# skovaka/UNCALLED

Measured on NVIDIA H100. Metric: reads/sec mapped (E. coli, 4k-sample reads) at 1/2/4/8 H100 vs CPU ref, higher is better.
Workload: dtype f32/f64 events, u32 FM index

## Files before the change

uncalled_b200/csrc/unc_device.cuh:

```cuda
#pragma once
#include "unc_warp.cuh"

typedef uint8_t u8;
typedef uint16_t u16;
typedef uint32_t u32;
typedef int32_t i32;
typedef uint64_t u64;

#define UNC_NKMER 1024
#define UNC_KMASK 0x3FFu
#define UNC_SEED_LEN 22u
#define UNC_NGEN 24u
#define UNC_PATH_MASK 0x3FFFFFu
#define UNC_PATH_TAIL 0x200000u
#define UNC_INVALID 0x80000000u
#define UNC_BLK 32u


struct DevIndex {
    const uint4 *bwt;
    const u32 *sa;
    const u32 *sa_full;
    const uint2 *kmer_range;
    const float *lv_mean, *lv_var2, *lognorm;
// ... 671 lines not shown
        t.len_sum = f_add(t.len_sum, (float) ns.total_len);
        if (ns.total_len >= p.min_map_len && ns.total_len > t.max_map.total_len) t.max_map = ns;
        trk_insert_unique(t, ns, have_lb ? &lb : nullptr);
    }
    PT_TRK(t, 2)
}

UNC_DEV bool trk_get_final(const Tracker &t, const DevParams &p) {
    if (t.max_map.total_len < p.min_map_len || t.n_lens < 2) return false;
    float mean_len = f_div(t.len_sum, (float) t.n_live);
    float second_len = (float) t.top2;
    float sl = (float) t.max_map.total_len;
    return (p.min_mean_conf > 0 && f_div(sl, mean_len) >= p.min_mean_conf) ||
           (p.min_top_conf > 0 && f_div(sl, second_len) >= p.min_top_conf);
}

#define K2_CH_SLOTS 160u
#define K2_V2_DYN_BYTES (16u + K2_MAXSEG * (K2_CH_SLOTS * 8u + K2_CH_SLOTS))
#ifndef K2_MAXSEG
#define K2_MAXSEG 16u
#endif
#define K2_DYN_PER_CHUNK 8u
#define K2_SMEM_BYTES(maxp) (sizeof(K2Shared) + 16 + (size_t) (((maxp) + 31) / 32) * K2_DYN_PER_CHUNK + 32 + K2_V2_DYN_BYTES)
struct K2Tables {
    uint2 kmer_range[UNC_NKMER];
    float thresh[64];
};
struct K2V2 {
    K2V2Tab t;
    u32 kcnt[UNC_NKMER];
    u32 koff[UNC_NKMER];
    u32 kagg[UNC_NKMER];
    u32 fresh_cand[32], fresh_mask[32], fresh_before[32];
    u32 grab[2];
    u32 n_units;
    u16 mfirst[K2V2_MAX_MERGED];
#if defined(UNC_PHASE_TIMING) && !defined(UNC_EMUL)
    u32 pt_dur[4][K2_MAXSEG];
#endif
};
struct K2Shared {
    K2Tables tb;
    float probs[UNC_NKMER];
    u32 flags[32];
    u32 flags_prev[32];
    u32 sort_hist[256 * K2_MAXSEG];
    uint4 trk_dir[1024];
    u32 *bcnt, *ecnt;
    K2V2 v2;
    unsigned char *v2_stage;
    u32 bc[8];
    u32 n_rows[2];
    u32 verdict[2];
    u32 wk_overflow;
    u32 wl_cnt;
    u32 cnt_blocks, cnt_steps;
    u32 tot_children[2], tot_sources[2];
    DevWork work;
};

#include "unc_pdqsort.cuh"
#ifdef UNC_EMUL
static unsigned long g_emu_tie_stats[2];
#endif
UNC_DEV void write_source(uint4 *rec, uint2 *hist_e, u32 idx, u32 st, u32 en, u32 kmer, float prob) {
    rec[(size_t) idx * 2] = make_uint4(st, en, kmer | (1u << 16), 1u);
    rec[(size_t) idx * 2 + 1] = make_uint4(f2u(prob), f2u(prob), 0u, 0u);
    hist_e[idx] = make_uint2(f2u(prob), 0xFFFFFFFFu);
// ... 49 lines not shown
                } else right = mid;
            }
            rid = mid;
        }
        u64 rf_st = 0, rf_len = 0;
        if (rid >= 0) { rf_st = sa_st - B.seq_offsets[rid]; rf_len = B.seq_lens[rid]; }
        o.mapped = 1; o.fwd = fwd ? 1 : 0; o.rid = rid;
        o.rf_st = rf_st; o.rf_len = rf_len;
        o.rf_en = rf_st + ((u64) sc.ren_end - (u64) sc.ref_st + 5u);
        o.matches = (sc.total_len + 4u) & 0xFFFFu;
    }
    o.n_children = ((u64) sh->tot_children[1] << 32) | sh->tot_children[0];
    o.n_sources = ((u64) sh->tot_sources[1] << 32) | sh->tot_sources[0];
    o.n_seeds = n_seeds;
    o.n_occ_blocks = sh->cnt_blocks; o.n_sa_steps = sh->cnt_steps;
    B.out[r] = o;
}

#if defined(UNC_PHASE_TIMING) && !defined(UNC_EMUL)
UNC_DEV long long pt_clock() { long long v; asm volatile("mov.u64 %0, %%clock64;" : "=l"(v) :: "memory"); return v; }
#define PT_DECL unsigned long long pt_acc[32]; for (int _i = 0; _i < 32; _i++) pt_acc[_i] = 0; long long pt_t = pt_clock();
#define UNC_PT_TRACE_READ 40u
#define UNC_PT_TRACE_E0 60u
#define UNC_PT_TRACE_BYTES (8u * 16u * 32u * 8u)
#define PT_TRACE(ev, i, t) if ((B).dbg && r == UNC_PT_TRACE_READ && (ev) - UNC_PT_TRACE_E0 < 8u && (c_tid() & 31) == 0) \
        (B).dbg[(size_t) (B).n_reads * 64 + ((size_t) ((ev) - UNC_PT_TRACE_E0) * 16 + (c_tid() >> 5)) * 32 + (i)] = (unsigned long long) (t);
#define PT_MARK(i) { long long _n = pt_clock(); pt_acc[i] += (unsigned long long) (_n - pt_t); pt_t = _n; PT_TRACE(event_i, i, _n) }
#define PT_FLUSH(B, r) if ((B).dbg && (wt == 0 || wt == nwt - 32u)) { for (int _i = 0; _i < (wt == 0 ? 32 : 28); _i++) (B).dbg[(size_t) (r) * 64 + (wt == 0 ? 0 : 32) + _i] = pt_acc[_i]; }
#define PT_FENCE c_sync_sub(1, (int) nwt);
#define PT_WDECL long long pt_w0 = 0;
#define PT_WB pt_w0 = pt_clock();
#define PT_WE(ph) if (lane == 0) v2->pt_dur[ph][ww] = (u32) (pt_clock() - pt_w0);
#define PT_WARR(ph) if (lane == 0) v2->pt_dur[ph][ww] = (u32) pt_clock(); w_sync(); s_atomic_max(&v2->pt_dur[ph][ww], (u32) pt_clock());
#define PT_WREL(ph) if (lane == 0 && *(volatile u32 *) &v2->grab[0] != 0xFFFFFFFFu) { const long long _t = pt_clock(); v2->pt_dur[ph][ww] = (u32) _t; PT_TRACE(event_i, 30, _t) }
#define PT_WLAG(ph, s_last, s_first) if (wt == 0) { const u32 _now = (u32) pt_clock(); u32 _mn = 0xFFFFFFFFu, _mx = 0; for (u32 _w = 0; _w < nwk; _w++) { \
        const u32 _d = _now - *(volatile u32 *) &v2->pt_dur[ph][_w]; _mn = _d < _mn ? _d : _mn; _mx = _d > _mx ? _d : _mx; } pt_acc[s_last] += _mn; pt_acc[s_first] += _mx; }
#define PT_WTRK(ph, s) if (wt == 0) pt_acc[s] += (u32) pt_clock() - *(volatile u32 *) &v2->pt_dur[ph][K2_MAXSEG - 2 + (event_i & 1u)];
#define PT_WR(ph, s_max, s_mean) if (wt == 0) { u32 _mx = 0, _sm = 0; for (u32 _w = 0; _w < nwk; _w++) { const u32 _d = *(volatile u32 *) &v2->pt_dur[ph][_w]; \
        _mx = _d > _mx ? _d : _mx; _sm += _d; } pt_acc[s_max] += _mx; pt_acc[s_mean] += _sm / nwk; }
#else
#define PT_DECL
#define PT_MARK(i)
#define PT_FLUSH(B, r)
#define PT_FENCE
#define PT_WDECL
#define PT_WB
#define PT_WE(ph)
#define PT_WARR(ph)
#define PT_WLAG(ph, s_last, s_first)
#define PT_WTRK(ph, s)
#define PT_WREL(ph)
#define PT_WR(ph, s_max, s_mean)
#endif

template <bool STREAM>
UNC_DEV void unc_k2_tracker(const DevIndex &ix, const DevParams &p, const DevBatch &B, const DevWork &W,
                            K2Shared *sh, u32 r, u32 n_first, u32 n_limit) {
    const int lane = w_lane();
    Tracker trk;
    trk.blocks = W.clu; trk.dir_glob = W.dir; trk.max_blocks = W.max_blocks;
    trk.dir = sh->trk_dir; trk.dir_cap = (u32) (sizeof(sh->trk_dir) / sizeof(uint4));
    trk_reset(trk);
    DevMapState *ms = nullptr;
    if (STREAM) {
        ms = B.mstate + B.chan[r];
        if (ms->started) {
            trk.nb = ms->t_nb; trk.n_alloc = ms->t_n_alloc; trk.n_live = ms->t_n_live; trk.n_lens = ms->t_n_lens;
// ... 147 lines not shown
```

uncalled_b200/csrc/unc_k2v2.cuh:

```cuda
#pragma once

#define K2V2_STAGE_BYTES (K2_CH_SLOTS * 8u + K2_CH_SLOTS)


UNC_DEV void unc_occ2_build_block(const uint4 *bwt, u32 j, uint4 *out) {
    const uint4 *p = bwt + ((size_t) (j >> 1) << 2);
    const uint4 b0 = p[0], b1 = p[1];
    uint4 cnt = make_uint4(b0.x, b0.z, b1.x, b1.z);
    const uint4 lo = p[2], hi = p[3];
    if (j & 1u) {
        const u32 w[4] = {lo.x, lo.y, lo.z, lo.w};
        for (int i = 0; i < 4; i++) {
            const u32 h = w[i] >> 1, m = 0x55555555u;
            const u32 c3 = (u32) d_popc(h & w[i] & m), c2 = (u32) d_popc(h & ~w[i] & m), c1 = (u32) d_popc(~h & w[i] & m);
            cnt.x += 16u - c1 - c2 - c3; cnt.y += c1; cnt.z += c2; cnt.w += c3;
        }
    }
    out[(size_t) j * 2] = cnt;
    out[(size_t) j * 2 + 1] = (j & 1u) ? hi : lo;
}

UNC_DEV void unc_occ2_all(const uint4 cnt, const uint4 sym, u32 p, u32 o[4]) {
    u32 c1 = 0, c2 = 0, c3 = 0;
#pragma unroll
// ... 90 lines not shown
                }
                src[j] = key;
            }
        }
        w_sync();
    }
}

struct K2V2Walk {
    bool dup, begin_v, after_v, seed;
    u32 as, ae;
    u32 m_b, m_a, m_seed;
};
UNC_DEV K2V2Walk k2v2_walk(const uint4 cur, u32 nx, u32 ny, bool a, bool has_next, bool head, bool first, bool use_carry,
                           u32 carry_mx, bool prob_ok, uint2 kr, u32 *mx_last) {
    const int lane = w_lane();
    K2V2Walk r;
    r.dup = has_next && nx == cur.x && ny == cur.y;
    u32 mx = a ? cur.y : 0u;
    bool hd = head || !a;
    for (int d = 1; d < 32; d <<= 1) {
        const u32 omx = w_shfl_up(mx, d), ohd = w_shfl_up(hd ? 1u : 0u, d);
        if (lane >= d && !hd) { mx = omx > mx ? omx : mx; hd = ohd != 0; }
    }
    if (use_carry) mx = mx > carry_mx ? mx : carry_mx;
    *mx_last = w_shfl(mx, 31);
    r.begin_v = a && first && prob_ok && kr.x <= cur.x - 1u;
    r.as = mx + 1u;
    r.ae = has_next ? nx - 1u : kr.y;
    r.after_v = a && !r.dup && prob_ok && r.as <= r.ae;
    r.seed = a && !r.dup && (cur.w & 1u);
    r.m_b = w_ballot(r.begin_v); r.m_a = w_ballot(r.after_v); r.m_seed = w_ballot(r.seed);
    return r;
}

struct K2V2Pack {
    bool a;
    u32 bl;
    u32 start, pos, n;
};
UNC_DEV K2V2Pack k2v2_next_pack(u32 cnt, u32 P, u32 *remaining) {
    const int lane = w_lane();
    const int s = d_ffs(*remaining) - 1;
    const u32 Ps = w_shfl(P, s);
    const bool fits = ((*remaining >> lane) & 1u) && (P + cnt - Ps <= 32u);
    const u32 in_pack = w_ballot(fits);
    *remaining &= ~in_pack;
    const int e = 31 - d_clz(in_pack);
    const u32 T = w_shfl(P + cnt, e) - Ps;
    K2V2Pack k;
    k.a = (u32) lane < T;
    k.bl = (u32) s; k.start = 0;
    u32 m = in_pack;
    while (m) {
        const int b = d_ffs(m) - 1;
        m &= m - 1;
        const u32 sb = w_shfl(P, b) - Ps;
        if ((u32) lane >= sb) { k.bl = (u32) b; k.start = sb; }
    }
    k.pos = (u32) lane - k.start;
    k.n = w_shfl(cnt, (int) k.bl);
    return k;
}
UNC_DEV u32 k2v2_segmask(u32 start, u32 n) { return (n >= 32u ? 0xFFFFFFFFu : ((1u << n) - 1u)) << start; }

UNC_DEV u32 k2v2_slot(u32 rank) { return ((rank & 31u) << 5) | (rank >> 5); }
// ... 1 lines not shown
UNC_DEV uint2 *k2v2_stage(K2Shared *sh, u32 ww) {
    const u32 off = (u32) (sh->v2_stage - (unsigned char *) sh) + ww * K2V2_STAGE_BYTES;
    return (uint2 *) ((unsigned char *) sh + off);
}

UNC_DEV void k2v2_add64(u32 *w, u32 v) {
    const u64 s = (((u64) w[1] << 32) | w[0]) + v;
    w[0] = (u32) s; w[1] = (u32) (s >> 32);
}

UNC_DEV u32 k2v2_grab(u32 *counter) {
    u32 g = 0;
    if (w_lane() == 0) g = s_atomic_add(counter, 1u);
    return w_shfl(g, 0);
}

UNC_DEV void k2v2_sort_small(uint4 *keys, u32 n, uint4 *sst) {
    const int lane = w_lane();
    const bool a = (u32) lane < n;
    uint4 k = make_uint4(0, 0, 0, 0);
    if (a) k = keys[lane];
    u32 rnk = 0;
    const u32 kf = k2v2_fkey(k.z), kr_ = k.w >> 14;
    for (u32 j = 0; j < n; j++) {
        const u32 jx = w_shfl(k.x, (int) j), jy = w_shfl(k.y, (int) j), jf = w_shfl(kf, (int) j), jr = w_shfl(kr_, (int) j);
        if (k2v2_less_pre(jx, jy, jf, jr, k.x, k.y, kf, kr_)) rnk++;
    }
    if (a) sst[rnk] = k;
    w_sync();
    if (a) keys[lane] = sst[lane];
    w_sync();
}

struct K2V2Emit {
    uint4 *next; uint2 *hist_e; u32 *onext; uint2 *rlist;
    u32 S0, nc, maxp, n_ended_rows, rl_cap, pos0;
    u32 src_before, seeds_before;
};
template <bool EMIT>
UNC_DEV u32 k2v2_walk_merged(const DevIndex &ix, K2Shared *sh, const uint4 *keys, u32 n, u32 moff, float source_prob,
                             const K2V2Emit &E, u32 *pend_steps, u32 *pend_blocks, uint4 *sst) {
    K2V2 *v2 = &sh->v2;
    const u32 lane = (u32) w_lane();
    u32 nsrc = 0, nseed = 0, prev_sub = 0xFFFFFFFFu, un_st = 1, un_en = 0;
  for (u32 g0 = 0; g0 < n; g0 += 32u) {
    const u32 cnt = n - g0 < 32u ? n - g0 : 32u;
    if (lane < cnt) sst[lane] = keys[g0 + lane];
    if (lane == 0 && g0 + cnt < n) sst[32] = keys[g0 + cnt];
    w_sync();
    if (lane == 0)
    for (u32 j = 0; j < cnt; j++) {
        const u32 i = g0 + j;
        const uint4 cur = sst[j];
        const u32 sub = (cur.w >> 6) & 0xFFu, kmer = v2->t.mk[moff + sub];
        const uint2 kr = sh->tb.kmer_range[kmer];
        const float pk = sh->probs[kmer];
        const bool ok = pk >= source_prob;
        if (sub != prev_sub) {
            if (!EMIT && v2->mfirst[moff + sub] == 0xFFFFu) v2->mfirst[moff + sub] = (u16) nsrc;
            if (ok) {
                if (kr.x <= cur.x - 1u) {
                    const u32 sidx = E.src_before + nsrc;
                    if (EMIT && E.nc + sidx < E.maxp) {
                        write_source(E.next, E.hist_e, E.S0 + E.nc + sidx, kr.x, cur.x - 1u, kmer, pk);
                        E.onext[E.nc + sidx] = E.S0 + E.nc + sidx;
                    }
                    nsrc++;
                }
                un_st = cur.y + 1u; un_en = kr.y;
            }
        }
        prev_sub = sub;
        const bool has_next = i + 1u < n;
        uint4 nxt = make_uint4(0, 0, 0, 0);
        if (has_next) nxt = sst[j + 1u];
        const bool dup = has_next && nxt.x == cur.x && nxt.y == cur.y;
        const u32 rec = cur.w >> 14;
        if (EMIT) E.onext[E.pos0 + i] = rec | (dup ? UNC_INVALID : 0u);
        if (dup) continue;
        if (ok) {
            u32 src_st = un_st, src_en = un_en;
            if (has_next && ((nxt.w >> 6) & 0xFFu) == sub) {
                src_en = nxt.x - 1u;
                if (un_st <= nxt.y) un_st = nxt.y + 1u;
            }
            if (src_st <= src_en) {
                const u32 sidx = E.src_before + nsrc;
                if (EMIT && E.nc + sidx < E.maxp) {
                    write_source(E.next, E.hist_e, E.S0 + E.nc + sidx, src_st, src_en, kmer, pk);
                    E.onext[E.nc + sidx] = E.S0 + E.nc + sidx;
                }
                nsrc++;
            }
        }
        if (cur.w & 1u) {
            if (EMIT) {
                d_atomic_or(&((u32 *) (E.next + (size_t) rec * 2))[3], 0x80000000u);
                const u32 ri = E.n_ended_rows + E.seeds_before + nseed;
                if (ri < E.rl_cap) E.rlist[ri] = make_uint2(ix.seq_len - unc_sa_lookup(ix, cur.x, pend_steps, pend_blocks), (cur.w >> 1) & 0x1Fu);
                else sh->wk_overflow = 1;
            }
            nseed++;
        }
    }
    w_sync();
  }
    return w_shfl(nsrc | (nseed << 16), 0);
}

UNC_DEV void k2v2_bucket_offsets(K2V2 *v2) {
    const u32 lane = (u32) w_lane();
    u32 sum = 0;
#pragma unroll 1
    for (u32 j = 0; j < 32; j++) sum += v2->kcnt[j * 32u + lane];
    u32 tot, run = w_exscan(sum, &tot);
#pragma unroll 1
    for (u32 j = 0; j < 32; j++) {
        const u32 sl = j * 32u + lane, v = v2->kcnt[sl];
        v2->koff[sl] = run;
        v2->kcnt[sl] = run;
        run += v;
    }
}

UNC_DEV bool k2v2_exact_order(K2Shared *sh, const DevWork &W, u32 nc, u32 maxp, u32 wt, u32 nwt) {
    uint4 *ckA = W.ckey, *ckB = W.ckey + maxp;
    for (u32 i = wt; i + 1u < nc; i += nwt) {
        const uint4 k0 = ckA[i], k1 = ckA[i + 1u];
        if (!pq_less(k0, k1) && !pq_less(k1, k0)) *(volatile u32 *) &sh->bc[5] = 1u;
    }
    c_sync_sub(1, (int) nwt);
#ifdef UNC_EMUL
    if (wt == 0) { g_emu_tie_stats[0]++; g_emu_tie_stats[1] += sh->bc[5]; }
#endif
    if (!*(volatile u32 *) &sh->bc[5]) return false;
    for (u32 i = wt; i < nc; i += nwt) {
        const uint4 k = ckA[i];
        const u32 ci = k.w >> 14;
        ckB[sh->bcnt[ci / K2_CH_SLOTS] + ci % K2_CH_SLOTS] = k;
    }
    c_sync_sub(1, (int) nwt);
    if (wt == 0 && !unc_pdq_sort(ckB, nc, W.cks, ((maxp + 31u) >> 5) * K2_CH_SLOTS)) s_atomic_or(&sh->wk_overflow, 1u);
    c_sync_sub(1, (int) nwt);
    for (u32 i = wt; i < nc; i += nwt) ckA[i] = ckB[i];
    K2V2 *v2 = &sh->v2;
    if (wt == 0) { v2->grab[0] = 0; v2->n_units = 0; }
    for (u32 m = wt; m < K2V2_MAX_MERGED; m += nwt) v2->mfirst[m] = 0xFFFFu;
    c_sync_sub(1, (int) nwt);
    return true;
}

template <bool STREAM, bool EXACT, bool FLAGS>
UNC_DEV void unc_k2_workers_v2(const DevIndex &ix, const DevParams &p, const DevBatch &B, const DevWork &W,
                               K2Shared *sh, u32 r, u32 n_first, u32 n_limit) {
    const int lane = w_lane();
    const u32 wt = (u32) c_tid() - 32u, nwt = (u32) c_nthreads() - 32u;
    const u32 ww = wt >> 5, nwk = nwt >> 5;
    const K2Tables *tb = &sh->tb;
    K2V2 *v2 = &sh->v2;
    const u32 maxp = p.max_paths;
    const u32 S0 = ((maxp + 31u) >> 5) * K2_CH_SLOTS;
    const size_t gen_recs = (size_t) S0 + maxp;
    const float source_prob = tb->thresh[0];
    u32 my_blocks = 0, my_steps = 0, pend_blocks = 0, pend_steps = 0;
    u32 prev_size = 0, gen = 0, event_i = n_first;
    if (STREAM) {
        const DevMapState *ms = B.mstate + B.chan[r];
        if (ms->started) { prev_size = ms->prev_size; gen = ms->gen; }
    }
    if (wt == 0) { sh->tot_children[0] = sh->tot_children[1] = 0; sh->tot_sources[0] = sh->tot_sources[1] = 0; }
    const u32 lt = w_lanemask_lt();
    PT_DECL
    PT_WDECL

    for (; event_i < n_limit; event_i++) {
        PT_MARK(9)
        const float event = f_add(f_mul(B.scale[r], B.events[(size_t) r * B.ev_stride + (event_i - n_first)]), B.shift[r]);
        PT_MARK(7)

        if (FLAGS && wt < 32u) sh->flags_prev[wt] = sh->flags[wt];
        for (u32 k = wt; k < UNC_NKMER; k += nwt) {
            sh->probs[k] = unc_match_prob(event, d_ldg(ix.lv_mean + k), d_ldg(ix.lv_var2 + k), d_ldg(ix.lognorm + k));
            v2->kcnt[k] = 0; v2->kagg[k] = 0;
        }
        for (u32 j = ww; j < 32; j += nwk) {
            const u32 k = j * 32 + (u32) lane;
            const float pk = unc_match_prob(event, d_ldg(ix.lv_mean + k), d_ldg(ix.lv_var2 + k), d_ldg(ix.lognorm + k));
            const uint2 kr = tb->kmer_range[k];
            const u32 m = w_ballot(pk >= source_prob && kr.x <= kr.y);
            if (lane == 0) v2->fresh_cand[j] = m;
        }
        if (wt == 0) { v2->grab[0] = 0; v2->grab[1] = 0; v2->n_units = 0; }
        if (EXACT && wt == 0) sh->bc[5] = 0;
        if (wt < K2V2_MAX_MERGED) v2->mfirst[wt] = 0xFFFFu;
        PT_MARK(0)
        c_sync_sub(1, (int) nwt);
        PT_FENCE
        PT_MARK(16)


        const u32 nch_prev = (prev_size + 31u) >> 5;
        {
            const uint4 *prev = W.paths + (size_t) gen * gen_recs * 2;
            uint4 *next = W.paths + (size_t) (gen ^ 1u) * gen_recs * 2, *cks = W.cks;
            uint2 *hist_e = W.hist + (size_t) (event_i % UNC_NGEN) * gen_recs;
            const u32 *oprev = W.order + (size_t) gen * maxp;
            uint2 *stage_r = k2v2_stage(sh, ww);
            u8 *stage_m = (u8 *) (stage_r + K2_CH_SLOTS);
            u32 oi_n = UNC_INVALID, oi_nn = UNC_INVALID; uint4 q0_n = make_uint4(0, 0, 0, 0); uint2 q1_n = make_uint2(0, 0);
            if (ww < nch_prev) {
                const u32 pi = ww * 32u + (u32) lane;
                if (pi < prev_size) oi_n = oprev[pi];
                if (!(oi_n & UNC_INVALID)) { const uint4 *pr = prev + (size_t) oi_n * 2; q0_n = pr[0]; q1_n = *(const uint2 *) (pr + 1); }
            }
            if (ww + nwk < nch_prev) {
                const u32 pi = (ww + nwk) * 32u + (u32) lane;
                if (pi < prev_size) oi_nn = oprev[pi];
                if (!(oi_nn & UNC_INVALID)) d_prefetch(prev + (size_t) oi_nn * 2);
            }
            for (u32 c = ww; c < nch_prev; c += nwk) {
                const u32 oi = oi_n;
                const uint4 q0 = q0_n; const uint2 q1 = q1_n;
                const bool valid = !(oi & UNC_INVALID);
                oi_n = oi_nn;
                if (c + nwk < nch_prev && !(oi_n & UNC_INVALID)) {
// ... 211 lines not shown
          {
            uint4 *ckA = W.ckey;
            const uint4 *cks = W.cks;
            uint4 kpre = make_uint4(0, 0, 0, 0);
            if (ww < nch_prev) {
                const u32 b0 = sh->bcnt[ww], e0 = ww + 1 < nch_prev ? sh->bcnt[ww + 1] : nc_total;
                if (b0 + (u32) lane < e0 && b0 + (u32) lane < nc) kpre = cks[(size_t) ww * K2_CH_SLOTS + (u32) lane];
            }
            for (u32 c = ww; c < nch_prev; c += nwk) {
                const u32 base = sh->bcnt[c];
                if (base >= nc) break;
                const u32 end = c + 1 < nch_prev ? sh->bcnt[c + 1] : nc_total;
                const uint4 kcur = kpre;
                if (c + nwk < nch_prev) {
                    const u32 bn = sh->bcnt[c + nwk], en = c + nwk + 1 < nch_prev ? sh->bcnt[c + nwk + 1] : nc_total;
                    if (bn + (u32) lane < en && bn + (u32) lane < nc) kpre = cks[(size_t) (c + nwk) * K2_CH_SLOTS + (u32) lane];
                }
                for (u32 i = (u32) lane; base + i < end && base + i < nc; i += 32) {
                    const u32 ci = c * K2_CH_SLOTS + i;
                    uint4 key = i < 32u ? kcur : cks[ci];
                    const u32 km = key.w & UNC_KMASK;
                    const u32 bk = v2->t.kslot[km];
                    key.w = ((key.w >> 10) & 0x3Fu) | ((u32) v2->t.ksub[km] << 6) | (ci << 14);
                    ckA[s_atomic_add(&v2->kcnt[bk], 1u)] = key;
                }
            }
          }
            PT_MARK(2)
            c_sync_sub(1, (int) nwt);
            PT_FENCE
            PT_MARK(18)
            PT_WB

            uint4 *csum = W.elist;
            uint4 *ckA = W.ckey, *ckB = W.ckey + maxp;
            uint2 *stage_r = k2v2_stage(sh, ww);
            u32 *whist = sh->sort_hist + (size_t) ww * 256u;
          for (bool recount = false;; recount = true) {
            const bool sort = !(EXACT && recount);
            for (;;) {
                const u32 gi = k2v2_grab(&v2->grab[0]);
                if (gi >= 96u) break;
                const u32 grp = gi & 31u;
                const u32 sl = (u32) lane * 32u + grp;
                const u32 bo = v2->koff[sl], bn = v2->kcnt[sl] - bo;
                const u32 meta = v2->t.gmeta[grp * 32u + (u32) lane];
                if (gi < 64u) {
                    const bool huge_sweep = gi < 32u;
                    u32 todo_m = huge_sweep ? w_ballot(meta != 0 && bn > 0) : 0u;
                    while (todo_m) {
                        const int l = d_ffs(todo_m) - 1;
                        todo_m &= todo_m - 1;
                        const u32 o = w_shfl(bo, l), n = w_shfl(bn, l), moff = w_shfl(meta, l) >> 8;
                        if (sort && n <= 32u) k2v2_sort_small(ckA + o, n, (uint4 *) stage_r);
                        else if (sort) {
                            u32 lo = 0xFFFFFFFFu, hi = 0;
                            for (u32 g = (u32) lane; g < n; g += 32u) { const u32 x = ckA[o + g].x; lo = x < lo ? x : lo; hi = x > hi ? x : hi; }
                            hi = w_max(hi);
                            lo = ~w_max(~lo);
                            k2v2_sort_big(ckA, ckB, o, n, lo, 32u - (u32) d_clz(hi - lo), whist);
                        }
                        {
                            K2V2Emit E;
                            E.src_before = 0; E.seeds_before = 0;
                            const u32 agg = k2v2_walk_merged<false>(ix, sh, ckA + o, n, moff, source_prob, E, &pend_steps, &pend_blocks, (uint4 *) stage_r);
                            if (lane == 0) v2->kagg[(u32) l * 32u + grp] = agg;
                        }
                    }
                    u32 todo = w_ballot(meta == 0 && (huge_sweep ? bn > 256u : (bn > 32u && bn <= 256u)));
                    while (todo) {
                        const int l = d_ffs(todo) - 1;
                        todo &= todo - 1;
                        const u32 o = w_shfl(bo, l), n = w_shfl(bn, l);
                        const u32 kmer = v2->t.gkmer[grp * 32u + (u32) l];
                        u32 ubase = 0;
                        if (lane == 0) ubase = s_atomic_add(&v2->n_units, (n + 31u) >> 5);
                        ubase = w_shfl(ubase, 0);
                        const uint2 kr = tb->kmer_range[kmer];
                        const bool prob_ok = sh->probs[kmer] >= source_prob;
                        if (sort) {
                            u32 lo = 0xFFFFFFFFu, hi = 0;
                            for (u32 g = (u32) lane; g < n; g += 32u) { const u32 x = ckA[o + g].x; lo = x < lo ? x : lo; hi = x > hi ? x : hi; }
                            hi = w_max(hi);
                            lo = ~w_max(~lo);
                            k2v2_sort_big(ckA, ckB, o, n, lo, 32u - (u32) d_clz(hi - lo), whist);
                        }
                        u32 carry_mx = 0, n_src = 0, n_seed = 0;
                        for (u32 g0 = 0; g0 < n; g0 += 32u) {
                            const u32 g = g0 + (u32) lane;
                            const bool a = g < n, has_next = g + 1u < n;
                            uint4 cur = make_uint4(0, 0, 0, 0); u32 nx = 0, ny = 0;
                            if (a) cur = ckA[o + g];
                            if (has_next) { const uint4 t = ckA[o + g + 1u]; nx = t.x; ny = t.y; }
                            if (lane == 0) csum[ubase + (g0 >> 5)] = make_uint4(carry_mx, n_src, n_seed, ((u32) l * 32u + grp) | ((g0 >> 5) << 10));
                            u32 mxo;
                            const K2V2Walk wk = k2v2_walk(cur, nx, ny, a, has_next, g == 0, g == 0, g0 != 0, carry_mx, prob_ok, kr, &mxo);
                            carry_mx = mxo;
                            n_src += (u32) d_popc(wk.m_b) + (u32) d_popc(wk.m_a);
                            n_seed += (u32) d_popc(wk.m_seed);
                        }
                        if (lane == 0) v2->kagg[(u32) l * 32u + grp] = n_src | (n_seed << 16);
                    }
                } else {
                    const u32 cnt = (bn > 0 && bn <= 32u && meta == 0) ? bn : 0u;
                    u32 tot;
                    const u32 P = w_exscan(cnt, &tot);
                    u32 remaining = w_ballot(cnt != 0);
                    while (remaining) {
                        const K2V2Pack pk = k2v2_next_pack(cnt, P, &remaining);
                        const u32 addr = w_shfl(bo, (int) pk.bl) + pk.pos;
                        uint4 k = make_uint4(0, 0, 0, 0);
                        if (pk.a) k = ckA[addr];
                        u32 rnk = pk.pos;
                        if (sort) {
                            const u32 maxn = w_max(pk.a ? pk.n : 0u);
                            rnk = 0;
                            const u32 kf = k2v2_fkey(k.z), kri = k.w >> 14;
                            for (u32 q = 0; q < maxn; q++) {
                                const int src = (int) ((pk.start + q) & 31u);
                                const u32 jx = w_shfl(k.x, src), jy = w_shfl(k.y, src), jf = w_shfl(kf, src), jr = w_shfl(kri, src);
                                if (pk.a && q < pk.n && k2v2_less_pre(jx, jy, jf, jr, k.x, k.y, kf, kri)) rnk++;
                            }
                        }
                        uint4 *sst = (uint4 *) stage_r;
                        if (pk.a) sst[pk.start + rnk] = k;
                        w_sync();
                        uint4 cur = make_uint4(0, 0, 0, 0);
                        if (pk.a) { cur = sst[lane]; ckA[addr] = cur; }
                        w_sync();
                        const u32 nx = w_shfl_down(cur.x, 1), ny = w_shfl_down(cur.y, 1);
                        const u32 kmer = v2->t.gkmer[grp * 32u + pk.bl];
                        const uint2 kr = tb->kmer_range[kmer];
                        const bool prob_ok = sh->probs[kmer] >= source_prob;
                        u32 mxo;
                        const K2V2Walk wk = k2v2_walk(cur, nx, ny, pk.a, pk.a && pk.pos + 1u < pk.n, pk.pos == 0, pk.pos == 0, false, 0u,
                                                      prob_ok, kr, &mxo);
                        const u32 sm = k2v2_segmask(pk.start, pk.n);
                        if (pk.a && pk.pos == 0)
                            v2->kagg[pk.bl * 32u + grp] = ((u32) d_popc(wk.m_b & sm) + (u32) d_popc(wk.m_a & sm)) | ((u32) d_popc(wk.m_seed & sm) << 16);
                    }
                }
            }
            PT_WE(1)
            PT_MARK(3)
            c_sync_sub(1, (int) nwt);
            if (!EXACT || recount || !k2v2_exact_order(sh, W, nc, maxp, wt, nwt)) break;
          }
            PT_FENCE
            PT_MARK(19)
            PT_WR(1, 15, 20)
        }

        if (ww == 0) {
            u32 sum = 0;
#pragma unroll 1
            for (u32 j = 0; j < 32; j++) sum += v2->kagg[j * 32u + (u32) lane];
            u32 ts, tq;
            const u32 es = w_exscan(sum & 0xFFFFu, &ts), eq = w_exscan(sum >> 16, &tq);
            u32 run = es | (eq << 16);
#pragma unroll 1
            for (u32 j = 0; j < 32; j++) {
                const u32 sl = j * 32u + (u32) lane, v = v2->kagg[sl];
                v2->kagg[sl] = run;
                if (nc > 0 && v2->kcnt[sl] != v2->koff[sl]) {
                    const u32 meta = v2->t.gmeta[(u32) lane * 32u + j];
                    if (meta == 0) {
                        const u32 kmer = v2->t.gkmer[(u32) lane * 32u + j];
                        if (sh->probs[kmer] >= source_prob && nc + (run & 0xFFFFu) < maxp) s_atomic_or(&sh->flags[kmer >> 5], 1u << (kmer & 31u));
                    } else {
                        for (u32 m = 0; m < (meta & 0xFFu); m++) {
// ... 8 lines not shown
            w_sync();
            const u32 tot_src = ts;
            const u32 ns_added = nc + tot_src > maxp ? maxp - nc : tot_src;
            const u32 nn0 = nc + ns_added;
            const u32 my_mask = v2->fresh_cand[lane] & ~sh->flags[lane];
            u32 tot_add;
            const u32 my_pre = w_exscan((u32) d_popc(my_mask), &tot_add);
            v2->fresh_mask[lane] = my_mask;
            v2->fresh_before[lane] = nn0 + my_pre;
            if (lane == 0) {
                sh->bc[1] = nn0 + tot_add < maxp ? nn0 + tot_add : maxp;
                sh->bc[6] = tq;
            }
        }
        if (ww != 0 || nwk == 1) {
            const u32 bt = nwk == 1 ? wt : wt - 32u, nbt = nwk == 1 ? nwt : nwt - 32u;
            uint2 *rlist = W.rlist + (size_t) (event_i & 1u) * W.rl_cap;
            for (u32 i = bt; i < n_ended_rows; i += nbt) {
                uint2 e = rlist[i];
                e.x = ix.seq_len - unc_sa_lookup(ix, e.x, &pend_steps, &pend_blocks);
                rlist[i] = e;
            }
        }
        PT_MARK(11)
        c_sync_sub(1, (int) nwt);
        PT_FENCE
        PT_MARK(27)
        PT_WB
        const u32 n_child_seeds = nc > 0 ? sh->bc[6] : 0u;
        n_rows = n_ended_rows + n_child_seeds;
        if (n_rows > W.rl_cap) n_rows = W.rl_cap;

        if (nc > 0) {
            const uint4 *csum = W.elist, *ckA = W.ckey;
            uint4 *next = W.paths + (size_t) (gen ^ 1u) * gen_recs * 2;
            uint2 *hist_e = W.hist + (size_t) (event_i % UNC_NGEN) * gen_recs;
            u32 *onext = W.order + (size_t) (gen ^ 1u) * maxp;
            uint2 *rlist = W.rlist + (size_t) (event_i & 1u) * W.rl_cap;
            uint2 *stage_r = k2v2_stage(sh, ww);
            const u32 n_units = *(volatile u32 *) &v2->n_units;
            for (;;) {
                const u32 gi = k2v2_grab(&v2->grab[1]);
                if (gi >= n_units + 32u) break;
                if (gi < n_units) {
                    const uint4 u = csum[gi];
                    const u32 sl_u = u.w & 1023u, g0 = (u.w >> 10) << 5;
                    const u32 o = v2->koff[sl_u], n = v2->kcnt[sl_u] - o, pre = v2->kagg[sl_u];
                    const u32 kmer = v2->t.gkmer[((sl_u & 31u) << 5) | (sl_u >> 5)];
                    const uint2 kr = tb->kmer_range[kmer];
                    const float pkm = sh->probs[kmer];
                    const bool prob_ok = pkm >= source_prob;
                    const u32 pos = g0 + (u32) lane;
                    const bool a = pos < n, has_next = pos + 1u < n;
                    uint4 cur = make_uint4(0, 0, 0, 0);
                    if (a) cur = ckA[o + pos];
                    u32 nx = w_shfl_down(cur.x, 1), ny = w_shfl_down(cur.y, 1);
                    if (lane == 31 && has_next) { const uint4 t = ckA[o + pos + 1u]; nx = t.x; ny = t.y; }
                    u32 mxo;
                    const K2V2Walk wk = k2v2_walk(cur, nx, ny, a, has_next, pos == 0, pos == 0, g0 != 0, u.x, prob_ok, kr, &mxo);
                    const u32 sidx = (pre & 0xFFFFu) + u.y + (u32) d_popc(wk.m_b & lt) + (u32) d_popc(wk.m_a & lt);
                    if (wk.begin_v && nc + sidx < maxp) {
                        write_source(next, hist_e, S0 + nc + sidx, kr.x, cur.x - 1u, kmer, pkm);
                        onext[nc + sidx] = S0 + nc + sidx;
                    }
                    const u32 sidx2 = sidx + (wk.begin_v ? 1u : 0u);
                    if (wk.after_v && nc + sidx2 < maxp) {
                        write_source(next, hist_e, S0 + nc + sidx2, wk.as, wk.ae, kmer, pkm);
                        onext[nc + sidx2] = S0 + nc + sidx2;
                    }
                    const u32 rec = cur.w >> 14;
                    if (a) onext[o + pos] = rec | (wk.dup ? UNC_INVALID : 0u);
                    if (wk.seed) {
                        d_atomic_or(&((u32 *) (next + (size_t) rec * 2))[3], 0x80000000u);
                        const u32 ri = n_ended_rows + (pre >> 16) + u.z + (u32) d_popc(wk.m_seed & lt);
                        if (ri < W.rl_cap)
                            rlist[ri] = make_uint2(ix.seq_len - unc_sa_lookup(ix, cur.x, &pend_steps, &pend_blocks), (cur.w >> 1) & 0x1Fu);
                        else sh->wk_overflow = 1;
                    }
                    continue;
                }
                const u32 grp = gi - n_units;
                const u32 sl = (u32) lane * 32u + grp;
                const u32 bo = v2->koff[sl], bn = v2->kcnt[sl] - bo, bpre = v2->kagg[sl];
                const u32 meta = v2->t.gmeta[grp * 32u + (u32) lane];
                u32 todo_m = w_ballot(meta != 0 && bn > 0);
                while (todo_m) {
                    const int l = d_ffs(todo_m) - 1;
                    todo_m &= todo_m - 1;
                    {
                        const u32 o_m = w_shfl(bo, l), n_m = w_shfl(bn, l), pre_m = w_shfl(bpre, l), mt_m = w_shfl(meta, l);
                        K2V2Emit E;
                        E.next = next; E.hist_e = hist_e; E.onext = onext; E.rlist = rlist;
                        E.S0 = S0; E.nc = nc; E.maxp = maxp; E.n_ended_rows = n_ended_rows; E.rl_cap = W.rl_cap; E.pos0 = o_m;
                        E.src_before = pre_m & 0xFFFFu; E.seeds_before = pre_m >> 16;
                        k2v2_walk_merged<true>(ix, sh, ckA + o_m, n_m, mt_m >> 8, source_prob, E, &pend_steps, &pend_blocks, (uint4 *) stage_r);
                    }
                }
                const u32 cnt = (bn > 0 && bn <= 32u && meta == 0) ? bn : 0u;
                u32 tot;
                const u32 P = w_exscan(cnt, &tot);
                u32 remaining = w_ballot(cnt != 0);
                while (remaining) {
                    const K2V2Pack pk = k2v2_next_pack(cnt, P, &remaining);
                    const u32 kmer = v2->t.gkmer[grp * 32u + pk.bl];
                    const uint2 kr = tb->kmer_range[kmer];
                    const float pkm = sh->probs[kmer];
                    const bool prob_ok = pkm >= source_prob;
                    const u32 pre = w_shfl(bpre, (int) pk.bl), o = w_shfl(bo, (int) pk.bl);
                    uint4 cur = make_uint4(0, 0, 0, 0);
                    if (pk.a) cur = ckA[o + pk.pos];
                    const u32 nx = w_shfl_down(cur.x, 1), ny = w_shfl_down(cur.y, 1);
                    u32 mxo;
                    const K2V2Walk wk = k2v2_walk(cur, nx, ny, pk.a, pk.a && pk.pos + 1u < pk.n, pk.pos == 0, pk.pos == 0, false, 0u, prob_ok,
                                                  kr, &mxo);
                    const u32 sm = k2v2_segmask(pk.start, pk.n);
                    const u32 sidx = (pre & 0xFFFFu) + (u32) d_popc(wk.m_b & lt & sm) + (u32) d_popc(wk.m_a & lt & sm);
                    if (wk.begin_v && nc + sidx < maxp) {
                        write_source(next, hist_e, S0 + nc + sidx, kr.x, cur.x - 1u, kmer, pkm);
                        onext[nc + sidx] = S0 + nc + sidx;
                    }
                    const u32 sidx2 = sidx + (wk.begin_v ? 1u : 0u);
                    if (wk.after_v && nc + sidx2 < maxp) {
                        write_source(next, hist_e, S0 + nc + sidx2, wk.as, wk.ae, kmer, pkm);
                        onext[nc + sidx2] = S0 + nc + sidx2;
                    }
                    const u32 rec = cur.w >> 14;
                    if (pk.a) onext[o + pk.pos] = rec | (wk.dup ? UNC_INVALID : 0u);
                    if (wk.seed) {
                        d_atomic_or(&((u32 *) (next + (size_t) rec * 2))[3], 0x80000000u);
                        const u32 ri = n_ended_rows + (pre >> 16) + (u32) d_popc(wk.m_seed & lt & sm);
                        if (ri < W.rl_cap)
                            rlist[ri] = make_uint2(ix.seq_len - unc_sa_lookup(ix, cur.x, &pend_steps, &pend_blocks), (cur.w >> 1) & 0x1Fu);
                        else sh->wk_overflow = 1;
                    }
                }
            }
        }
        PT_WE(2)
        uint4 *next = W.paths + (size_t) (gen ^ 1u) * gen_recs * 2;
        uint2 *hist_e = W.hist + (size_t) (event_i % UNC_NGEN) * gen_recs;
        u32 *onext = W.order + (size_t) (gen ^ 1u) * maxp;
        for (u32 j = ww; j < 32; j += nwk) {
            const u32 before = v2->fresh_before[j];
            if (before >= maxp) continue;
            const u32 k = j * 32 + (u32) lane;
            const u32 fw = sh->flags[j];
            u32 m_add = v2->fresh_mask[j];
            const u32 room = maxp - before;
            u32 visited = 0xFFFFFFFFu;
            if ((u32) d_popc(m_add) >= room) {
                u32 mm = m_add;
                for (u32 q = 1; q < room; q++) mm &= mm - 1;
                int last = d_ffs(mm) - 1;
                visited = last == 31 ? 0xFFFFFFFFu : ((2u << last) - 1u);
                m_add &= visited;
            }
            const u32 rank = (u32) d_popc(m_add & lt);
            if ((m_add >> lane) & 1u) {
                const uint2 kr = tb->kmer_range[k];
                write_source(next, hist_e, S0 + before + rank, kr.x, kr.y, k, sh->probs[k]);
                onext[before + rank] = S0 + before + rank;
            }
            w_sync();
            if (lane == 0) sh->flags[j] = fw & ~visited;
        }
        if (wt == 0) *(volatile u32 *) &sh->n_rows[event_i & 1u] = n_rows;
        PT_WARR(3)
// ... 29 lines not shown
```

Before: 5246.

## Record per-candidate verdicts in first pass and emit with flat parallel loop

The first walk pass now stores a per-candidate verdict record (flags, source bounds, local prefix counts, kmer, slot) into the spare ckB buffer. The second emit pass no longer re-walks every group with work-stealing grabs and warp scans. Instead all threads run one strided loop over candidates, combining the stored verdict with the per-slot aggregate to write sources, order entries and seeds. This removes the duplicated walk computation, the unit-summary buffer and the second grab counter, at the cost of an extra 16-byte write and read per candidate.

```diff
diff --git a/uncalled_b200/csrc/unc_device.cuh b/uncalled_b200/csrc/unc_device.cuh
--- a/uncalled_b200/csrc/unc_device.cuh
+++ b/uncalled_b200/csrc/unc_device.cuh
@@ -727,8 +727,7 @@
     u32 koff[UNC_NKMER];
     u32 kagg[UNC_NKMER];
     u32 fresh_cand[32], fresh_mask[32], fresh_before[32];
-    u32 grab[2];
-    u32 n_units;
+    u32 grab;
     u16 mfirst[K2V2_MAX_MERGED];
 #if defined(UNC_PHASE_TIMING) && !defined(UNC_EMUL)
     u32 pt_dur[4][K2_MAXSEG];
@@ -844,7 +843,7 @@
 #define PT_WB pt_w0 = pt_clock();
 #define PT_WE(ph) if (lane == 0) v2->pt_dur[ph][ww] = (u32) (pt_clock() - pt_w0);
 #define PT_WARR(ph) if (lane == 0) v2->pt_dur[ph][ww] = (u32) pt_clock(); w_sync(); s_atomic_max(&v2->pt_dur[ph][ww], (u32) pt_clock());
-#define PT_WREL(ph) if (lane == 0 && *(volatile u32 *) &v2->grab[0] != 0xFFFFFFFFu) { const long long _t = pt_clock(); v2->pt_dur[ph][ww] = (u32) _t; PT_TRACE(event_i, 30, _t) }
+#define PT_WREL(ph) if (lane == 0 && *(volatile u32 *) &v2->grab != 0xFFFFFFFFu) { const long long _t = pt_clock(); v2->pt_dur[ph][ww] = (u32) _t; PT_TRACE(event_i, 30, _t) }
 #define PT_WLAG(ph, s_last, s_first) if (wt == 0) { const u32 _now = (u32) pt_clock(); u32 _mn = 0xFFFFFFFFu, _mx = 0; for (u32 _w = 0; _w < nwk; _w++) { \
         const u32 _d = _now - *(volatile u32 *) &v2->pt_dur[ph][_w]; _mn = _d < _mn ? _d : _mn; _mx = _d > _mx ? _d : _mx; } pt_acc[s_last] += _mn; pt_acc[s_first] += _mx; }
 #define PT_WTRK(ph, s) if (wt == 0) pt_acc[s] += (u32) pt_clock() - *(volatile u32 *) &v2->pt_dur[ph][K2_MAXSEG - 2 + (event_i & 1u)];
diff --git a/uncalled_b200/csrc/unc_k2v2.cuh b/uncalled_b200/csrc/unc_k2v2.cuh
--- a/uncalled_b200/csrc/unc_k2v2.cuh
+++ b/uncalled_b200/csrc/unc_k2v2.cuh
@@ -146,6 +146,17 @@
     r.seed = a && !r.dup && (cur.w & 1u);
     r.m_b = w_ballot(r.begin_v); r.m_a = w_ballot(r.after_v); r.m_seed = w_ballot(r.seed);
     return r;
+}
+
+#define K2V2_V_DUP 1u
+#define K2V2_V_BEGIN 2u
+#define K2V2_V_AFTER 4u
+#define K2V2_V_SEED 8u
+UNC_DEV uint4 k2v2_verdict(u32 as, u32 ae, u32 before, u32 flags, u32 kmer, u32 slot) {
+    return make_uint4(as, ae, before, flags | (kmer << 4) | (slot << 14));
+}
+UNC_DEV u32 k2v2_flags(const K2V2Walk &w) {
+    return (w.dup ? K2V2_V_DUP : 0u) | (w.begin_v ? K2V2_V_BEGIN : 0u) | (w.after_v ? K2V2_V_AFTER : 0u) | (w.seed ? K2V2_V_SEED : 0u);
 }
 
 struct K2V2Pack {
@@ -213,14 +224,8 @@
     w_sync();
 }
 
-struct K2V2Emit {
-    uint4 *next; uint2 *hist_e; u32 *onext; uint2 *rlist;
-    u32 S0, nc, maxp, n_ended_rows, rl_cap, pos0;
-    u32 src_before, seeds_before;
-};
-template <bool EMIT>
-UNC_DEV u32 k2v2_walk_merged(const DevIndex &ix, K2Shared *sh, const uint4 *keys, u32 n, u32 moff, float source_prob,
-                             const K2V2Emit &E, u32 *pend_steps, u32 *pend_blocks, uint4 *sst) {
+UNC_DEV u32 k2v2_walk_merged(K2Shared *sh, const uint4 *keys, uint4 *verd, u32 n, u32 moff, u32 slot, float source_prob,
+                             uint4 *sst) {
     K2V2 *v2 = &sh->v2;
     const u32 lane = (u32) w_lane();
     u32 nsrc = 0, nseed = 0, prev_sub = 0xFFFFFFFFu, un_st = 1, un_en = 0;
@@ -235,19 +240,13 @@
         const uint4 cur = sst[j];
         const u32 sub = (cur.w >> 6) & 0xFFu, kmer = v2->t.mk[moff + sub];
         const uint2 kr = sh->tb.kmer_range[kmer];
-        const float pk = sh->probs[kmer];
-        const bool ok = pk >= source_prob;
+        const bool ok = sh->probs[kmer] >= source_prob;
+        const u32 before = nsrc | (nseed << 16);
+        u32 fl = 0, src_st = 0, src_en = 0;
         if (sub != prev_sub) {
-            if (!EMIT && v2->mfirst[moff + sub] == 0xFFFFu) v2->mfirst[moff + sub] = (u16) nsrc;
+            if (v2->mfirst[moff + sub] == 0xFFFFu) v2->mfirst[moff + sub] = (u16) nsrc;
             if (ok) {
-                if (kr.x <= cur.x - 1u) {
-                    const u32 sidx = E.src_before + nsrc;
-                    if (EMIT && E.nc + sidx < E.maxp) {
-                        write_source(E.next, E.hist_e, E.S0 + E.nc + sidx, kr.x, cur.x - 1u, kmer, pk);
-                        E.onext[E.nc + sidx] = E.S0 + E.nc + sidx;
-                    }
-                    nsrc++;
-                }
+                if (kr.x <= cur.x - 1u) { fl |= K2V2_V_BEGIN; nsrc++; }
                 un_st = cur.y + 1u; un_en = kr.y;
             }
         }
@@ -255,34 +254,19 @@
         const bool has_next = i + 1u < n;
         uint4 nxt = make_uint4(0, 0, 0, 0);
         if (has_next) nxt = sst[j + 1u];
-        const bool dup = has_next && nxt.x == cur.x && nxt.y == cur.y;
-        const u32 rec = cur.w >> 14;
-        if (EMIT) E.onext[E.pos0 + i] = rec | (dup ? UNC_INVALID : 0u);
-        if (dup) continue;
-        if (ok) {
-            u32 src_st = un_st, src_en = un_en;
-            if (has_next && ((nxt.w >> 6) & 0xFFu) == sub) {
-                src_en = nxt.x - 1u;
-                if (un_st <= nxt.y) un_st = nxt.y + 1u;
-            }
-            if (src_st <= src_en) {
-                const u32 sidx = E.src_before + nsrc;
-                if (EMIT && E.nc + sidx < E.maxp) {
-                    write_source(E.next, E.hist_e, E.S0 + E.nc + sidx, src_st, src_en, kmer, pk);
-                    E.onext[E.nc + sidx] = E.S0 + E.nc + sidx;
-                }
-                nsrc++;
-            }
-        }
-        if (cur.w & 1u) {
-            if (EMIT) {
-                d_atomic_or(&((u32 *) (E.next + (size_t) rec * 2))[3], 0x80000000u);
-                const u32 ri = E.n_ended_rows + E.seeds_before + nseed;
-                if (ri < E.rl_cap) E.rlist[ri] = make_uint2(ix.seq_len - unc_sa_lookup(ix, cur.x, pend_steps, pend_blocks), (cur.w >> 1) & 0x1Fu);
-                else sh->wk_overflow = 1;
-            }
-            nseed++;
-        }
+        if (has_next && nxt.x == cur.x && nxt.y == cur.y) fl |= K2V2_V_DUP;
+        else {
+            if (ok) {
+                src_st = un_st; src_en = un_en;
+                if (has_next && ((nxt.w >> 6) & 0xFFu) == sub) {
+                    src_en = nxt.x - 1u;
+                    if (un_st <= nxt.y) un_st = nxt.y + 1u;
+                }
+                if (src_st <= src_en) { fl |= K2V2_V_AFTER; nsrc++; }
+            }
+            if (cur.w & 1u) { fl |= K2V2_V_SEED; nseed++; }
+        }
+        verd[i] = k2v2_verdict(src_st, src_en, before, fl, kmer, slot);
     }
     w_sync();
   }
@@ -325,7 +309,7 @@
     c_sync_sub(1, (int) nwt);
     for (u32 i = wt; i < nc; i += nwt) ckA[i] = ckB[i];
     K2V2 *v2 = &sh->v2;
-    if (wt == 0) { v2->grab[0] = 0; v2->n_units = 0; }
+    if (wt == 0) v2->grab = 0;
     for (u32 m = wt; m < K2V2_MAX_MERGED; m += nwt) v2->mfirst[m] = 0xFFFFu;
     c_sync_sub(1, (int) nwt);
     return true;
@@ -371,7 +355,7 @@
             const u32 m = w_ballot(pk >= source_prob && kr.x <= kr.y);
             if (lane == 0) v2->fresh_cand[j] = m;
         }
-        if (wt == 0) { v2->grab[0] = 0; v2->grab[1] = 0; v2->n_units = 0; }
+        if (wt == 0) v2->grab = 0;
         if (EXACT && wt == 0) sh->bc[5] = 0;
         if (wt < K2V2_MAX_MERGED) v2->mfirst[wt] = 0xFFFFu;
         PT_MARK(0)
@@ -649,14 +633,13 @@
             PT_MARK(18)
             PT_WB
 
-            uint4 *csum = W.elist;
             uint4 *ckA = W.ckey, *ckB = W.ckey + maxp;
             uint2 *stage_r = k2v2_stage(sh, ww);
             u32 *whist = sh->sort_hist + (size_t) ww * 256u;
           for (bool recount = false;; recount = true) {
             const bool sort = !(EXACT && recount);
             for (;;) {
-                const u32 gi = k2v2_grab(&v2->grab[0]);
+                const u32 gi = k2v2_grab(&v2->grab);
                 if (gi >= 96u) break;
                 const u32 grp = gi & 31u;
                 const u32 sl = (u32) lane * 32u + grp;
@@ -677,22 +660,16 @@
                             lo = ~w_max(~lo);
                             k2v2_sort_big(ckA, ckB, o, n, lo, 32u - (u32) d_clz(hi - lo), whist);
                         }
-                        {
-                            K2V2Emit E;
-                            E.src_before = 0; E.seeds_before = 0;
-                            const u32 agg = k2v2_walk_merged<false>(ix, sh, ckA + o, n, moff, source_prob, E, &pend_steps, &pend_blocks, (uint4 *) stage_r);
-                            if (lane == 0) v2->kagg[(u32) l * 32u + grp] = agg;
-                        }
+                        const u32 slot = (u32) l * 32u + grp;
+                        const u32 agg = k2v2_walk_merged(sh, ckA + o, ckB + o, n, moff, slot, source_prob, (uint4 *) stage_r);
+                        if (lane == 0) v2->kagg[slot] = agg;
                     }
                     u32 todo = w_ballot(meta == 0 && (huge_sweep ? bn > 256u : (bn > 32u && bn <= 256u)));
                     while (todo) {
                         const int l = d_ffs(todo) - 1;
                         todo &= todo - 1;
                         const u32 o = w_shfl(bo, l), n = w_shfl(bn, l);
-                        const u32 kmer = v2->t.gkmer[grp * 32u + (u32) l];
-                        u32 ubase = 0;
-                        if (lane == 0) ubase = s_atomic_add(&v2->n_units, (n + 31u) >> 5);
-                        ubase = w_shfl(ubase, 0);
+                        const u32 kmer = v2->t.gkmer[grp * 32u + (u32) l], slot = (u32) l * 32u + grp;
                         const uint2 kr = tb->kmer_range[kmer];
                         const bool prob_ok = sh->probs[kmer] >= source_prob;
                         if (sort) {
@@ -709,14 +686,17 @@
                             uint4 cur = make_uint4(0, 0, 0, 0); u32 nx = 0, ny = 0;
                             if (a) cur = ckA[o + g];
                             if (has_next) { const uint4 t = ckA[o + g + 1u]; nx = t.x; ny = t.y; }
-                            if (lane == 0) csum[ubase + (g0 >> 5)] = make_uint4(carry_mx, n_src, n_seed, ((u32) l * 32u + grp) | ((g0 >> 5) << 10));
                             u32 mxo;
                             const K2V2Walk wk = k2v2_walk(cur, nx, ny, a, has_next, g == 0, g == 0, g0 != 0, carry_mx, prob_ok, kr, &mxo);
                             carry_mx = mxo;
+                            if (a) {
+                                const u32 src_b = n_src + (u32) d_popc(wk.m_b & lt) + (u32) d_popc(wk.m_a & lt), seed_b = n_seed + (u32) d_popc(wk.m_seed & lt);
+                                ckB[o + g] = k2v2_verdict(wk.as, wk.ae, src_b | (seed_b << 16), k2v2_flags(wk), kmer, slot);
+                            }
                             n_src += (u32) d_popc(wk.m_b) + (u32) d_popc(wk.m_a);
                             n_seed += (u32) d_popc(wk.m_seed);
                         }
-                        if (lane == 0) v2->kagg[(u32) l * 32u + grp] = n_src | (n_seed << 16);
+                        if (lane == 0) v2->kagg[slot] = n_src | (n_seed << 16);
                     }
                 } else {
                     const u32 cnt = (bn > 0 && bn <= 32u && meta == 0) ? bn : 0u;
@@ -753,6 +733,10 @@
                         const K2V2Walk wk = k2v2_walk(cur, nx, ny, pk.a, pk.a && pk.pos + 1u < pk.n, pk.pos == 0, pk.pos == 0, false, 0u,
                                                       prob_ok, kr, &mxo);
                         const u32 sm = k2v2_segmask(pk.start, pk.n);
+                        if (pk.a) {
+                            const u32 src_b = (u32) d_popc(wk.m_b & lt & sm) + (u32) d_popc(wk.m_a & lt & sm), seed_b = (u32) d_popc(wk.m_seed & lt & sm);
+                            ckB[addr] = k2v2_verdict(wk.as, wk.ae, src_b | (seed_b << 16), k2v2_flags(wk), kmer, pk.bl * 32u + grp);
+                        }
                         if (pk.a && pk.pos == 0)
                             v2->kagg[pk.bl * 32u + grp] = ((u32) d_popc(wk.m_b & sm) + (u32) d_popc(wk.m_a & sm)) | ((u32) d_popc(wk.m_seed & sm) << 16);
                     }
@@ -827,107 +811,38 @@
         if (n_rows > W.rl_cap) n_rows = W.rl_cap;
 
         if (nc > 0) {
-            const uint4 *csum = W.elist, *ckA = W.ckey;
+            const uint4 *ckA = W.ckey, *verd = W.ckey + maxp;
             uint4 *next = W.paths + (size_t) (gen ^ 1u) * gen_recs * 2;
             uint2 *hist_e = W.hist + (size_t) (event_i % UNC_NGEN) * gen_recs;
             u32 *onext = W.order + (size_t) (gen ^ 1u) * maxp;
             uint2 *rlist = W.rlist + (size_t) (event_i & 1u) * W.rl_cap;
-            uint2 *stage_r = k2v2_stage(sh, ww);
-            const u32 n_units = *(volatile u32 *) &v2->n_units;
-            for (;;) {
-                const u32 gi = k2v2_grab(&v2->grab[1]);
-                if (gi >= n_units + 32u) break;
-                if (gi < n_units) {
-                    const uint4 u = csum[gi];
-                    const u32 sl_u = u.w & 1023u, g0 = (u.w >> 10) << 5;
-                    const u32 o = v2->koff[sl_u], n = v2->kcnt[sl_u] - o, pre = v2->kagg[sl_u];
-                    const u32 kmer = v2->t.gkmer[((sl_u & 31u) << 5) | (sl_u >> 5)];
-                    const uint2 kr = tb->kmer_range[kmer];
+            for (u32 i = wt; i < nc; i += nwt) {
+                const uint4 cur = ckA[i], v = verd[i];
+                const u32 rec = cur.w >> 14;
+                onext[i] = rec | ((v.w & K2V2_V_DUP) ? UNC_INVALID : 0u);
+                if (!(v.w & (K2V2_V_BEGIN | K2V2_V_AFTER | K2V2_V_SEED))) continue;
+                const u32 kmer = (v.w >> 4) & 1023u, pre = v2->kagg[v.w >> 14];
+                if (v.w & (K2V2_V_BEGIN | K2V2_V_AFTER)) {
                     const float pkm = sh->probs[kmer];
-                    const bool prob_ok = pkm >= source_prob;
-                    const u32 pos = g0 + (u32) lane;
-                    const bool a = pos < n, has_next = pos + 1u < n;
-                    uint4 cur = make_uint4(0, 0, 0, 0);
-                    if (a) cur = ckA[o + pos];
-                    u32 nx = w_shfl_down(cur.x, 1), ny = w_shfl_down(cur.y, 1);
-                    if (lane == 31 && has_next) { const uint4 t = ckA[o + pos + 1u]; nx = t.x; ny = t.y; }
-                    u32 mxo;
-                    const K2V2Walk wk = k2v2_walk(cur, nx, ny, a, has_next, pos == 0, pos == 0, g0 != 0, u.x, prob_ok, kr, &mxo);
-                    const u32 sidx = (pre & 0xFFFFu) + u.y + (u32) d_popc(wk.m_b & lt) + (u32) d_popc(wk.m_a & lt);
-                    if (wk.begin_v && nc + sidx < maxp) {
-                        write_source(next, hist_e, S0 + nc + sidx, kr.x, cur.x - 1u, kmer, pkm);
+                    u32 sidx = (pre & 0xFFFFu) + (v.z & 0xFFFFu);
+                    if (v.w & K2V2_V_BEGIN) {
+                        if (nc + sidx < maxp) {
+                            write_source(next, hist_e, S0 + nc + sidx, tb->kmer_range[kmer].x, cur.x - 1u, kmer, pkm);
+                            onext[nc + sidx] = S0 + nc + sidx;
+                        }
+                        sidx++;
+                    }
+                    if ((v.w & K2V2_V_AFTER) && nc + sidx < maxp) {
+                        write_source(next, hist_e, S0 + nc + sidx, v.x, v.y, kmer, pkm);
                         onext[nc + sidx] = S0 + nc + sidx;
                     }
-                    const u32 sidx2 = sidx + (wk.begin_v ? 1u : 0u);
-                    if (wk.after_v && nc + sidx2 < maxp) {
-                        write_source(next, hist_e, S0 + nc + sidx2, wk.as, wk.ae, kmer, pkm);
-                        onext[nc + sidx2] = S0 + nc + sidx2;
-                    }
-                    const u32 rec = cur.w >> 14;
-                    if (a) onext[o + pos] = rec | (wk.dup ? UNC_INVALID : 0u);
-                    if (wk.seed) {
-                        d_atomic_or(&((u32 *) (next + (size_t) rec * 2))[3], 0x80000000u);
-                        const u32 ri = n_ended_rows + (pre >> 16) + u.z + (u32) d_popc(wk.m_seed & lt);
-                        if (ri < W.rl_cap)
-                            rlist[ri] = make_uint2(ix.seq_len - unc_sa_lookup(ix, cur.x, &pend_steps, &pend_blocks), (cur.w >> 1) & 0x1Fu);
-                        else sh->wk_overflow = 1;
-                    }
-                    continue;
-                }
-                const u32 grp = gi - n_units;
-                const u32 sl = (u32) lane * 32u + grp;
-                const u32 bo = v2->koff[sl], bn = v2->kcnt[sl] - bo, bpre = v2->kagg[sl];
-                const u32 meta = v2->t.gmeta[grp * 32u + (u32) lane];
-                u32 todo_m = w_ballot(meta != 0 && bn > 0);
-                while (todo_m) {
-                    const int l = d_ffs(todo_m) - 1;
-                    todo_m &= todo_m - 1;
-                    {
-                        const u32 o_m = w_shfl(bo, l), n_m = w_shfl(bn, l), pre_m = w_shfl(bpre, l), mt_m = w_shfl(meta, l);
-                        K2V2Emit E;
-                        E.next = next; E.hist_e = hist_e; E.onext = onext; E.rlist = rlist;
-                        E.S0 = S0; E.nc = nc; E.maxp = maxp; E.n_ended_rows = n_ended_rows; E.rl_cap = W.rl_cap; E.pos0 = o_m;
-                        E.src_before = pre_m & 0xFFFFu; E.seeds_before = pre_m >> 16;
-                        k2v2_walk_merged<true>(ix, sh, ckA + o_m, n_m, mt_m >> 8, source_prob, E, &pend_steps, &pend_blocks, (uint4 *) stage_r);
-                    }
-                }
-                const u32 cnt = (bn > 0 && bn <= 32u && meta == 0) ? bn : 0u;
-                u32 tot;
-                const u32 P = w_exscan(cnt, &tot);
-                u32 remaining = w_ballot(cnt != 0);
-                while (remaining) {
-                    const K2V2Pack pk = k2v2_next_pack(cnt, P, &remaining);
-                    const u32 kmer = v2->t.gkmer[grp * 32u + pk.bl];
-                    const uint2 kr = tb->kmer_range[kmer];
-                    const float pkm = sh->probs[kmer];
-                    const bool prob_ok = pkm >= source_prob;
-                    const u32 pre = w_shfl(bpre, (int) pk.bl), o = w_shfl(bo, (int) pk.bl);
-                    uint4 cur = make_uint4(0, 0, 0, 0);
-                    if (pk.a) cur = ckA[o + pk.pos];
-                    const u32 nx = w_shfl_down(cur.x, 1), ny = w_shfl_down(cur.y, 1);
-                    u32 mxo;
-                    const K2V2Walk wk = k2v2_walk(cur, nx, ny, pk.a, pk.a && pk.pos + 1u < pk.n, pk.pos == 0, pk.pos == 0, false, 0u, prob_ok,
-                                                  kr, &mxo);
-                    const u32 sm = k2v2_segmask(pk.start, pk.n);
-                    const u32 sidx = (pre & 0xFFFFu) + (u32) d_popc(wk.m_b & lt & sm) + (u32) d_popc(wk.m_a & lt & sm);
-                    if (wk.begin_v && nc + sidx < maxp) {
-                        write_source(next, hist_e, S0 + nc + sidx, kr.x, cur.x - 1u, kmer, pkm);
-                        onext[nc + sidx] = S0 + nc + sidx;
-                    }
-                    const u32 sidx2 = sidx + (wk.begin_v ? 1u : 0u);
-                    if (wk.after_v && nc + sidx2 < maxp) {
-                        write_source(next, hist_e, S0 + nc + sidx2, wk.as, wk.ae, kmer, pkm);
-                        onext[nc + sidx2] = S0 + nc + sidx2;
-                    }
-                    const u32 rec = cur.w >> 14;
-                    if (pk.a) onext[o + pk.pos] = rec | (wk.dup ? UNC_INVALID : 0u);
-                    if (wk.seed) {
-                        d_atomic_or(&((u32 *) (next + (size_t) rec * 2))[3], 0x80000000u);
-                        const u32 ri = n_ended_rows + (pre >> 16) + (u32) d_popc(wk.m_seed & lt & sm);
-                        if (ri < W.rl_cap)
-                            rlist[ri] = make_uint2(ix.seq_len - unc_sa_lookup(ix, cur.x, &pend_steps, &pend_blocks), (cur.w >> 1) & 0x1Fu);
-                        else sh->wk_overflow = 1;
-                    }
+                }
+                if (v.w & K2V2_V_SEED) {
+                    d_atomic_or(&((u32 *) (next + (size_t) rec * 2))[3], 0x80000000u);
+                    const u32 ri = n_ended_rows + (pre >> 16) + (v.z >> 16);
+                    if (ri < W.rl_cap)
+                        rlist[ri] = make_uint2(ix.seq_len - unc_sa_lookup(ix, cur.x, &pend_steps, &pend_blocks), (cur.w >> 1) & 0x1Fu);
+                    else sh->wk_overflow = 1;
                 }
             }
         }
```

After: 5468 (median of 6 runs). 4.2% higher.
